# MohamedAbou-Taleb/Iterative-Linear-Quadratic-Regulator

Hardware: AMD Instinct MI355X
Metric: iLQR iterations/sec (batch=4096, T=200, n=4 m=1); backward-pass HBM GB/s (higher is better)
Workload: dtype f32; 1 GPU; c3: under-actuated double pendulum swing-up (run_iLQR_UA_MPC.py params), n=4 m=1 N=200 rk4, batch 4096 trajectories per GPU, 10 parallel line-search alphas per pass covering the 10 reference trials, fixed iterations; batch_per_gpu=4096, horizon=200, n_alpha=10, n_trials=10

## Files before the change

iterative-linear-quadratic-regulator_amd/csrc/backward_tile16.hpp:

```cpp
#pragma once
#include <type_traits>
#include <utility>

#include "dynamics.hpp"

namespace ilqr {

constexpr int dpp_quad(int a, int b, int c, int d) { return a | (b << 2) | (c << 4) | (d << 6); }
constexpr int kRowRor = 0x120;
constexpr int kDown1 = kRowRor + 12;
constexpr int kDown2 = kRowRor + 8;
constexpr int kDown3 = kRowRor + 4;
constexpr int kRight1 = dpp_quad(1, 2, 3, 0);
constexpr int kRight2 = dpp_quad(2, 3, 0, 1);
constexpr int kRight3 = dpp_quad(3, 0, 1, 2);
constexpr int kSwap1 = dpp_quad(1, 0, 3, 2);

template <int CTRL, int BANK = 0xf, bool BOUND = true> ILQR_DEV int dpp_bits(int old, int v) {
    return __builtin_amdgcn_update_dpp(old, v, CTRL, 0xf, BANK, BOUND);
}
template <int CTRL> ILQR_DEV float dpp(float v) {
    return __int_as_float(dpp_bits<CTRL>(0, __float_as_int(v)));
}
template <int CTRL> ILQR_DEV double dpp(double v) {
    const int lo = dpp_bits<CTRL>(0, __double2loint(v));
    const int hi = dpp_bits<CTRL>(0, __double2hiint(v));
    return __hiloint2double(hi, lo);
}
template <int CTRL, int BANK> ILQR_DEV float dpp_row(float old, float v) {
    return __int_as_float(dpp_bits<CTRL, BANK, false>(__float_as_int(old), __float_as_int(v)));
}
template <int CTRL, int BANK> ILQR_DEV double dpp_row(double old, double v) {
    const int lo = dpp_bits<CTRL, BANK, false>(__double2loint(old), __double2loint(v));
    const int hi = dpp_bits<CTRL, BANK, false>(__double2hiint(old), __double2hiint(v));
    return __hiloint2double(hi, lo);
}

template <typename T> struct Vec4;
template <> struct Vec4<float> { using type = float4; };
template <> struct Vec4<double> { using type = double4; };

constexpr int kTile16 = 48;

constexpr int kTileAux = ILQR_NT_TILE_LOAD ? 2 : 0;
typedef unsigned int u32x4 __attribute__((ext_vector_type(4)));
typedef unsigned int u32x2 __attribute__((ext_vector_type(2)));
ILQR_DEV int uniform(int v) { return __builtin_amdgcn_readfirstlane(v); }
ILQR_DEV __amdgpu_buffer_rsrc_t make_rsrc(const void* base, unsigned bytes) {
    const unsigned long long a = (unsigned long long)base;
    const unsigned lo = (unsigned)uniform((int)(unsigned)a), hi = (unsigned)uniform((int)(unsigned)(a >> 32));
    void* ub = (void*)(((unsigned long long)hi << 32) | lo);
    return __builtin_amdgcn_make_buffer_rsrc(ub, 0, (unsigned)uniform((int)bytes), 0x00020000);
}
template <int IMM, typename T> struct BufLoad;
template <int IMM> struct BufLoad<IMM, float> {
    static ILQR_DEV void v4(__amdgpu_buffer_rsrc_t r, int voff, int soff, float* o) {
        const u32x4 v = __builtin_amdgcn_raw_buffer_load_b128(r, voff + IMM * 4, soff, kTileAux);
        o[0] = __uint_as_float(v.x); o[1] = __uint_as_float(v.y); o[2] = __uint_as_float(v.z); o[3] = __uint_as_float(v.w);
    }
    static ILQR_DEV float v1(__amdgpu_buffer_rsrc_t r, int voff, int soff) {
        return __uint_as_float(__builtin_amdgcn_raw_buffer_load_b32(r, voff + IMM * 4, soff, kTileAux));
    }
};
template <int IMM> struct BufLoad<IMM, double> {
    static ILQR_DEV void v4(__amdgpu_buffer_rsrc_t r, int voff, int soff, double* o) {
        const u32x4 a = __builtin_amdgcn_raw_buffer_load_b128(r, voff + IMM * 8, soff, kTileAux);
        const u32x4 b = __builtin_amdgcn_raw_buffer_load_b128(r, voff + IMM * 8 + 16, soff, kTileAux);
        o[0] = __hiloint2double((int)a.y, (int)a.x); o[1] = __hiloint2double((int)a.w, (int)a.z);
        o[2] = __hiloint2double((int)b.y, (int)b.x); o[3] = __hiloint2double((int)b.w, (int)b.z);
    }
    static ILQR_DEV double v1(__amdgpu_buffer_rsrc_t r, int voff, int soff) {
        const u32x2 a = __builtin_amdgcn_raw_buffer_load_b64(r, voff + IMM * 8, soff, kTileAux);
        return __hiloint2double((int)a.y, (int)a.x);
    }
};
ILQR_DEV void buf_store1(__amdgpu_buffer_rsrc_t r, int voff, int soff, float v) {
    __builtin_amdgcn_raw_buffer_store_b32(__float_as_uint(v), r, voff, soff, 0);
}
ILQR_DEV void buf_store1(__amdgpu_buffer_rsrc_t r, int voff, int soff, double v) {
    u32x2 w = {(unsigned)__double2loint(v), (unsigned)__double2hiint(v)};
    __builtin_amdgcn_raw_buffer_store_b64(w, r, voff, soff, 0);
}

template <typename T, int C, bool NOP2 = false> ILQR_DEV void buf_store_vec(__amdgpu_buffer_rsrc_t r, int voff, int soff, const T* v) {
    constexpr int BYTES = C * (int)sizeof(T), PB = BYTES % 16 == 0 ? 16 : BYTES % 8 == 0 ? 8 : 4, NP = BYTES / PB;
    unsigned w[BYTES / 4];
    __builtin_memcpy(w, v, BYTES);
#pragma unroll
    for (int k = 0; k < NP; ++k) {
        if constexpr (PB == 16) {
            const u32x4 q = {w[4 * k], w[4 * k + 1], w[4 * k + 2], w[4 * k + 3]};
            __builtin_amdgcn_raw_buffer_store_b128(q, r, voff + 16 * k, soff, 0);
            if constexpr (NOP2) asm volatile("s_nop 1" : : "v"(q));
            else asm volatile("s_nop 0" : : "v"(q));
        } else if constexpr (PB == 8) {
            const u32x2 q = {w[2 * k], w[2 * k + 1]};
            __builtin_amdgcn_raw_buffer_store_b64(q, r, voff + 8 * k, soff, 0);
        } else {
            __builtin_amdgcn_raw_buffer_store_b32(w[k], r, voff + 4 * k, soff, 0);
        }
    }
}

struct TileOffsets { int vi, vj, vl; };

template <typename T> struct Tile16 {
    T ski[4];
    T skj[4];
    T vj[4];
    T lxx;
    T bi;
    T luxi;
};

template <typename T> ILQR_DEV void tile16_load(Tile16<T>& tl, const T* __restrict__ tp, int i, int j, int l16) {
    using V4 = typename Vec4<T>::type;
    const V4 a = *reinterpret_cast<const V4*>(tp + 4 * i);
    const V4 c = *reinterpret_cast<const V4*>(tp + 4 * j);
    const V4 v = *reinterpret_cast<const V4*>(tp + 32 + 4 * j);
    tl.ski[0] = a.x; tl.ski[1] = a.y; tl.ski[2] = a.z; tl.ski[3] = a.w;
    tl.skj[0] = c.x; tl.skj[1] = c.y; tl.skj[2] = c.z; tl.skj[3] = c.w;
    tl.vj[0] = v.x; tl.vj[1] = v.y; tl.vj[2] = v.z; tl.vj[3] = v.w;
    tl.lxx = tp[16 + l16];
    tl.bi = tp[32 + 4 * i];
    tl.luxi = tp[32 + 4 * i + 2];
}

template <typename T>
ILQR_DEV void tile16_load_buf(Tile16<T>& tl, __amdgpu_buffer_rsrc_t r, const TileOffsets& o, int soff) {
    BufLoad<0, T>::v4(r, o.vi, soff, tl.ski);
    BufLoad<0, T>::v4(r, o.vj, soff, tl.skj);
    BufLoad<32, T>::v4(r, o.vj, soff, tl.vj);
    tl.lxx = BufLoad<16, T>::v1(r, o.vl, soff);
    tl.bi = BufLoad<32, T>::v1(r, o.vi, soff);
    tl.luxi = BufLoad<34, T>::v1(r, o.vi, soff);
}

struct TileQ {
    float skj[4];
    float vj[4];
    float a;
    float lxx;
    float c;
};
ILQR_DEV void tileq_load_buf(TileQ& tl, __amdgpu_buffer_rsrc_t r, const TileOffsets& o, int soff) {
    BufLoad<0, float>::v4(r, o.vj, soff, tl.skj);
    BufLoad<32, float>::v4(r, o.vj, soff, tl.vj);
    tl.a = BufLoad<0, float>::v1(r, o.vl, soff);
    tl.lxx = BufLoad<16, float>::v1(r, o.vl, soff);
    tl.c = BufLoad<32, float>::v1(r, o.vl, soff);
}

#if ILQR_NT_TILE_LOAD
#define ILQR_TILE_NT " nt"
#else
#define ILQR_TILE_NT ""
#endif
typedef int i32x4 __attribute__((ext_vector_type(4)));
typedef float f32x4n __attribute__((ext_vector_type(4)));
typedef double f64x2n __attribute__((ext_vector_type(2)));

ILQR_DEV i32x4 make_srd(const void* base, unsigned bytes) {
    const unsigned long long a = (unsigned long long)base;
    i32x4 d;
    d.x = uniform((int)(unsigned)a);
    d.y = uniform((int)((unsigned)(a >> 32) & 0xffffu));
    d.z = uniform((int)bytes);
    d.w = 0x00020000;
    return d;
}

template <int... I, typename F> ILQR_DEV void static_for_impl(std::integer_sequence<int, I...>, F&& f) {
    (f(std::integral_constant<int, I>{}), ...);
}
template <int N, typename F> ILQR_DEV void static_for(F&& f) {
    static_for_impl(std::make_integer_sequence<int, N>{}, f);
}

template <typename T> struct RawTile;
#define ILQR_OUT_FIRST(x) "=&v"(x)
#define ILQR_OUT_REFILL(x) "+&v"(x)
template <> struct RawTile<float> {
    static constexpr int NLOAD = 5;
    f32x4n ski, skj, vj, vi;
    float lxx;
#define ILQR_RAWTILE_F32(OUT)                                                                \
    asm volatile(                                                                            \
        "s_nop 4\n\t"                                                                        \
        "buffer_load_dwordx4 %0, %5, %8, %9 offen" ILQR_TILE_NT "\n\t"                       \
        "buffer_load_dwordx4 %1, %6, %8, %9 offen" ILQR_TILE_NT "\n\t"                       \
        "buffer_load_dwordx4 %2, %6, %8, %9 offen offset:128" ILQR_TILE_NT "\n\t"            \
        "buffer_load_dword %3, %7, %8, %9 offen offset:64" ILQR_TILE_NT "\n\t"               \
        "buffer_load_dwordx4 %4, %5, %8, %9 offen offset:128" ILQR_TILE_NT                   \
        : OUT(ski), OUT(skj), OUT(vj), OUT(lxx), OUT(vi)                                     \
        : "v"(o.vi), "v"(o.vj), "v"(o.vl), "s"(srd), "s"(soff)                               \
        : "memory")
    template <bool FIRST> ILQR_DEV void issue(const i32x4& srd, const TileOffsets& o, int soff) {
        if constexpr (FIRST) ILQR_RAWTILE_F32(ILQR_OUT_FIRST);
        else ILQR_RAWTILE_F32(ILQR_OUT_REFILL);
    }
    template <int N> ILQR_DEV void wait() {
        asm volatile("s_waitcnt vmcnt(%5)" : "+v"(ski), "+v"(skj), "+v"(vj), "+v"(lxx), "+v"(vi) : "i"(N) : "memory");
    }
    ILQR_DEV void unpack(Tile16<float>& t) const {
        t.ski[0] = ski.x; t.ski[1] = ski.y; t.ski[2] = ski.z; t.ski[3] = ski.w;
// ... 599 lines not shown
```

iterative-linear-quadratic-regulator_amd/csrc/kernels.hpp:

```cpp
#pragma once
#include "dynamics.hpp"

namespace ilqr {

#ifndef ILQR_NT_TILE_STORE
#define ILQR_NT_TILE_STORE 0
#endif
#ifndef ILQR_NT_TILE_LOAD
#define ILQR_NT_TILE_LOAD 0
#endif
#ifndef ILQR_DROP_ALL
#define ILQR_DROP_ALL 0
#endif
constexpr int kMaxAlpha = 16;
constexpr int kCounterRing = 64;
constexpr int kBoxMaxU = 2;
constexpr int kALMaxX = 4;

template <typename T> struct Limits {
    T u_lo[kBoxMaxU], u_hi[kBoxMaxU];
    T x_lo[kALMaxX], x_hi[kALMaxX];
    int al_mask;
    const T* u_lo_rows;
    const T* u_hi_rows;
    const T* x_lo_rows;
    const T* x_hi_rows;
};

template <typename T> struct KArgs {
    int B, N, n_slots, integ, maxiter, flags;
    int n_pass;
    int last_pass;
    int init_mode;
    int counter_idx;
    T dt, tol, mu;
    T alphas[kMaxAlpha];
    T* X; T* U; int* cur_slot;
    T* gains; T* lin; T* term; T* x0;
    T* costs; T* cost; T* cost_prev; T* alpha_taken;
    int* status; int* iters; int* accepted; int* counters;
    int reset_slots;
    int const_lin;
    int fuse_select;
    int lin_sparse;
    int t_first;
    const T* params;
    long long* probe;
    alignas(sizeof(T)) int box;
    alignas(sizeof(T)) int het;
    const T* rows;
    const T* plant_rows;
    const T* lam;
    const T* rho;
    Limits<T> lim;
};

template <int NU, typename T> ILQR_DEV void box_bounds(const Limits<T>& a, size_t B, int b, T* lo, T* hi) {
    const T* __restrict__ rl = a.u_lo_rows;
    const T* __restrict__ rh = a.u_hi_rows;
#pragma unroll
    for (int j = 0; j < NU; ++j) {
        lo[j] = rl ? rl[(size_t)j * B + b] : a.u_lo[j];
        hi[j] = rl ? rh[(size_t)j * B + b] : a.u_hi[j];
    }
}

template <int NH, typename T> ILQR_DEV void load_row(T* p, const T* __restrict__ rows, size_t B, int b) {
#pragma unroll
    for (int q = 0; q < NH; ++q) p[q] = rows[(size_t)q * B + b];
}

constexpr int gain_record(int nx, int nu) { return ((nu * nx + nu) + 3) / 4 * 4; }

ILQR_DEV bool traj_active(int status) { return (status & 0xff) == ILQR_TRAJ_ACTIVE; }

template <typename T> ILQR_DEV T clamp_keep_nan(T v, T lo, T hi) { return v < lo ? lo : (v > hi ? hi : v); }

ILQR_DEV size_t vec_at(size_t B, int Tn, int C, int slot, int t, size_t b) {
    return ((((size_t)slot * Tn + t) * B) + b) * C;
}
typedef unsigned int vec_u4 __attribute__((ext_vector_type(4)));
typedef unsigned int vec_u2 __attribute__((ext_vector_type(2)));
constexpr int vec_piece(int bytes) { return bytes % 16 == 0 ? 16 : bytes % 8 == 0 ? 8 : 4; }
constexpr int vec_pieces(int bytes) { return bytes / vec_piece(bytes); }
template <typename T, int C> ILQR_DEV void vec_load(const T* __restrict__ p, T* o) {
    constexpr int BYTES = C * (int)sizeof(T), PB = vec_piece(BYTES), NP = BYTES / PB;
    if constexpr (PB == 16) {
        vec_u4 v[NP];
#pragma unroll
        for (int k = 0; k < NP; ++k) v[k] = reinterpret_cast<const vec_u4*>(p)[k];
        __builtin_memcpy(o, v, BYTES);
    } else if constexpr (PB == 8) {
        vec_u2 v[NP];
#pragma unroll
        for (int k = 0; k < NP; ++k) v[k] = reinterpret_cast<const vec_u2*>(p)[k];
        __builtin_memcpy(o, v, BYTES);
    } else {
#pragma unroll
        for (int i = 0; i < C; ++i) o[i] = p[i];
    }
}
template <typename T, int C> ILQR_DEV void vec_store(T* __restrict__ p, const T* v) {
    constexpr int BYTES = C * (int)sizeof(T), PB = vec_piece(BYTES), NP = BYTES / PB;
    if constexpr (PB == 16) {
        vec_u4 w[NP];
        __builtin_memcpy(w, v, BYTES);
#pragma unroll
        for (int k = 0; k < NP; ++k) reinterpret_cast<vec_u4*>(p)[k] = w[k];
    } else if constexpr (PB == 8) {
        vec_u2 w[NP];
        __builtin_memcpy(w, v, BYTES);
#pragma unroll
        for (int k = 0; k < NP; ++k) reinterpret_cast<vec_u2*>(p)[k] = w[k];
    } else {
#pragma unroll
        for (int i = 0; i < C; ++i) p[i] = v[i];
    }
}

struct ClockProbe {
    long long c0, r0;
    ILQR_DEV void start() { c0 = __builtin_readcyclecounter(); r0 = wall_clock64(); }
    ILQR_DEV void stop(long long* probe, int slot) const {
        if (probe && threadIdx.x == 0) {
            const long long c1 = __builtin_readcyclecounter(), r1 = wall_clock64();
            const size_t wg = (size_t)blockIdx.y * gridDim.x + blockIdx.x;
            if (wg == 0) { probe[2 * slot] = c1 - c0; probe[2 * slot + 1] = r1 - r0; }
            if (wg < 65536) {
                long long* q = probe + 8 + ((size_t)slot * 65536 + wg) * 4;
                q[0] = r0; q[1] = r1; q[2] = c1 - c0;
                q[3] = (long long)__builtin_amdgcn_s_getreg((4 ) | (0 << 6) | (31 << 11)) |
                       ((long long)__builtin_amdgcn_s_getreg((20 ) | (0 << 6) | (3 << 11)) << 32);
            }
        }
    }
};

}
#include "backward_tile16.hpp"
#include "backward_tile16m2.hpp"
namespace ilqr {

template <typename TS, int NX, int NU, typename T, typename Pick>
ILQR_DEV void tile16_fill(Pick pick, const T (*fx)[NX], const T (*fu)[NU], const T* gxn, const T* gu1, const T (*lxxn)[NX],
                          const T (*luxn)[NX], const T (*luu)[NU], typename Vec4<TS>::type* tile) {
    static_assert((NX >= 2 && NX <= 4 && NU == 1) || (NX == 4 && NU == 2), "tile packing: n_x <= 4 with n_u = 1, or (4, 2)");
    auto F = [&](int i, int j) -> TS { return (i < NX && j < NX) ? pick(fx[i < NX ? i : 0][j < NX ? j : 0]) : TS(0); };
    auto L = [&](int i, int j) -> TS { return (i < NX && j < NX) ? pick(lxxn[i < NX ? i : 0][j < NX ? j : 0]) : TS(0); };
#pragma unroll
    for (int c = 0; c < 4; ++c) {
        tile[c].x = F((c + 0) & 3, c); tile[c].y = F((c + 1) & 3, c);
        tile[c].z = F((c + 2) & 3, c); tile[c].w = F((c + 3) & 3, c);
    }
#pragma unroll
// ... 600 lines not shown
    if (a.reset_slots) a.cur_slot[b] = 0;
    const size_t B = a.B;
    T Vx[NX], Vxx[NX][NX];
    load_terminal<T, NX>(a.term, B, b, Vx, Vxx);
    bool all_pd = true;
    T blo[NU], bhi[NU];
    box_bounds<NU>(a.lim, a.B, b, blo, bhi);
    for (int t = a.N - 1; t >= 0; --t) {
        T tile[E], u[NU];
        load_expansion<E>(a.lin + ((size_t)t * E) * B + b, B, tile);
        vec_load<T, NU>(a.U + vec_at(B, a.N, NU, slot, t, b), u);
        T Qx[NX], Qu[NU], Qxx[NX][NX], Qux[NU][NX], Quu[NU][NU], Qr[NU][NU];
        riccati_q<T, NX, NU>(tile, Vx, Vxx, Qx, Qu, Qxx, Qux, Quu);
#pragma unroll
        for (int i = 0; i < NU; ++i)
#pragma unroll
            for (int j = 0; j < NU; ++j) Qr[i][j] = Quu[i][j] + ((i == j) ? a.mu : T(0));
        T K[NU][NX], k[NU], lo[NU], hi[NU];
        const bool pd = gain_solve<T, NX, NU>(Qr, Qux, Qu, K, k);
        all_pd = all_pd && pd;
#pragma unroll
        for (int i = 0; i < NU; ++i) {
            lo[i] = blo[i] - u[i];
            hi[i] = bhi[i] - u[i];
        }
        const bool moved = box_gains<T, NX, NU>(Qr, Qux, Qu, lo, hi, pd, K, k);
        riccati_value<T, NX, NU>(moved || a.mu != T(0), Qx, Qu, Qxx, Qux, Quu, K, k, Vx, Vxx);
        constexpr int R = gain_record(NX, NU);
        store_gains<T, NX, NU>(a.gains + ((size_t)t * B + b) * R, K, k);
    }
    if (!all_pd) a.status[b] = st | ILQR_TRAJ_FLAG_NON_PD;
}

template <typename T, typename Dyn, int INTEG, bool BOX, bool HET = false, bool AL = false>
ILQR_DEV void forward_body(const KArgs<T>& a) {
    constexpr int NX = Dyn::NX, NU = Dyn::NU;
    constexpr int R = gain_record(NX, NU);
    const int b = blockIdx.x * blockDim.x + threadIdx.x;
    const int ai = blockIdx.y;
    if (a.init_mode && blockIdx.x == 0 && ai == 0 && threadIdx.x == 0) a.counters[a.counter_idx] = 0;
    if (b >= a.B) return;
    if (!a.init_mode) {
        if (!traj_active(a.status[b])) return;
        if (a.accepted[b]) return;
    }
    const size_t B = a.B;
    const int N = a.N;
    const int slot = a.cur_slot[b];
    const int cslot = (slot + 1 + ai) % a.n_slots;
    const T alpha = a.alphas[ai];
    using PLf = ParamLayout<Dyn::NSYS, NX, NU>;
    T ph[HET ? PLf::QS : 1];
    if constexpr (HET) {
#pragma unroll
        for (int i = 0; i < PLf::QS; ++i) ph[i] = a.params[i];
        load_row<PLf::Q>(ph, a.rows, B, b);
    }
    const T* __restrict__ p = HET ? ph : a.params;
    T x[NX], u[NU];
#pragma unroll
    for (int i = 0; i < NX; ++i) x[i] = a.x0[(size_t)i * B + b];
    ClockProbe cp;
    cp.start();
    T cost = T(0);
    const T* Xo = a.X + vec_at(B, N + 1, NX, slot, 0, b);
    const T* Uo = a.U + vec_at(B, N, NU, slot, 0, b);
    const T* G = a.gains + (size_t)b * R;
    T* Xc = a.X + vec_at(B, N + 1, NX, cslot, 0, b);
    T* Uc = a.U + vec_at(B, N, NU, cslot, 0, b);
    const size_t sX = B * NX, sU = B * NU;
    constexpr bool PREFETCH = (R <= 32);
    constexpr int RN = PREFETCH ? R : 1, NXN = PREFETCH ? NX : 1, NUN = PREFETCH ? NU : 1;
    T xo[NX], uo[NU], g[R], xo_n[NXN], uo_n[NUN], g_n[RN];
    vec_load<T, NX>(Xo, xo);
    vec_load<T, NU>(Uo, uo);
#pragma unroll
    for (int r = 0; r < R; ++r) g[r] = G[r];
    constexpr int NL = AL ? 2 * NX : 1;
    T lam[NL], lam_n[NL];
    const T rho = AL ? a.rho[b] : T(0);
    T blo[BOX ? NU : 1], bhi[BOX ? NU : 1];
    if constexpr (BOX) box_bounds<NU>(a.lim, a.B, b, blo, bhi);
    struct NoBounds { ILQR_DEV NoBounds(const Limits<T>&, size_t, int) {} };
    const std::conditional_t<AL, ALBounds<T, NX>, NoBounds> xb(a.lim, a.B, b);
    for (int t = 0; t < N; ++t) {
        const int tn = (t + 1 < N) ? t + 1 : t;
        if constexpr (PREFETCH) {
            vec_load<T, NX>(Xo + tn * sX, xo_n);
            vec_load<T, NU>(Uo + tn * sU, uo_n);
#pragma unroll
            for (int r = 0; r < R; ++r) g_n[r] = G[(size_t)tn * B * R + r];
        }
        T dx[NX];
#pragma unroll
        for (int i = 0; i < NX; ++i) dx[i] = x[i] - xo[i];
#pragma unroll
        for (int j = 0; j < NU; ++j) {
            T fb = T(0);
#pragma unroll
            for (int i = 0; i < NX; ++i) fb += g[j * NX + i] * dx[i];
            u[j] = uo[j] + alpha * g[NU * NX + j] + fb;
            if constexpr (BOX) u[j] = clamp_keep_nan(u[j], blo[j], bhi[j]);
        }
        vec_store<T, NX>(Xc + t * sX, x);
        vec_store<T, NU>(Uc + t * sU, u);
        cost += Cost<T, Dyn>::stage(p, a.dt, x, u);
        if constexpr (AL) {
            if (t > 0) cost += al_phi<T, NX>(xb, x, lam, rho);
            al_load_lam<T, NX>(a, B, b, t + 1, lam_n);
        }
        T xn[NX];
        Stepper<T, Dyn>::step(INTEG, p, a.dt, x, u, xn);
#pragma unroll
        for (int i = 0; i < NX; ++i) x[i] = xn[i];
        if constexpr (AL) {
#pragma unroll
            for (int q = 0; q < NL; ++q) lam[q] = lam_n[q];
        }
        if constexpr (PREFETCH) {
#pragma unroll
            for (int i = 0; i < NX; ++i) xo[i] = xo_n[i];
#pragma unroll
            for (int j = 0; j < NU; ++j) uo[j] = uo_n[j];
#pragma unroll
            for (int r = 0; r < R; ++r) g[r] = g_n[r];
        } else {
            vec_load<T, NX>(Xo + tn * sX, xo);
            vec_load<T, NU>(Uo + tn * sU, uo);
#pragma unroll
            for (int r = 0; r < R; ++r) g[r] = G[(size_t)tn * B * R + r];
        }
    }
    vec_store<T, NX>(Xc + N * sX, x);
    cost += Cost<T, Dyn>::terminal(p, x);
    if constexpr (AL) cost += al_phi<T, NX>(xb, x, lam, rho);
    a.costs[(size_t)ai * B + b] = cost;
    cp.stop(a.probe, 1);
}
template <typename T, typename Dyn, int INTEG>
__global__ void __launch_bounds__(64) forward_kernel(KArgs<T> a) { forward_body<T, Dyn, INTEG, false>(a); }
template <typename T, typename Dyn, int INTEG>
__global__ void __launch_bounds__(64) forward_kernel_box(KArgs<T> a) { forward_body<T, Dyn, INTEG, true>(a); }
template <typename T, typename Dyn, int INTEG>
__global__ void __launch_bounds__(64) forward_kernel_het(KArgs<T> a) { forward_body<T, Dyn, INTEG, false, true>(a); }
template <typename T, typename Dyn, int INTEG>
__global__ void __launch_bounds__(64) forward_kernel_box_het(KArgs<T> a) { forward_body<T, Dyn, INTEG, true, true>(a); }
template <typename T, typename Dyn, int INTEG>
__global__ void __launch_bounds__(64) forward_kernel_al(KArgs<T> a) { forward_body<T, Dyn, INTEG, true, false, true>(a); }
template <typename T, typename Dyn, int INTEG>
__global__ void __launch_bounds__(64) forward_kernel_al_het(KArgs<T> a) { forward_body<T, Dyn, INTEG, true, true, true>(a); }

#include "fwd_in_gen.inc"

template <typename T, typename Dyn, int INTEG, bool BOX = false, bool HET = false>
ILQR_DEV void rollout_ring(const KArgs<T>& a, int b, int ai, bool in_range, bool force_init = false) {
    constexpr int NX = Dyn::NX, NU = Dyn::NU;
    using In = FwdIn<T, NX, NU>;
    constexpr int R = In::R, NLD = In::NLD, NST = vec_pieces(NX * (int)sizeof(T)) + vec_pieces(NU * (int)sizeof(T));
#ifndef ILQR_RING_PF_MAX
#define ILQR_RING_PF_MAX 6
#endif
    constexpr int SLOT_REGS = (NX + NU + R) * (int)sizeof(T) / 4;
    constexpr int PF_CNT = (63 / (NLD + NST)) + 1 > ILQR_RING_PF_MAX ? ILQR_RING_PF_MAX : (63 / (NLD + NST)) + 1;
    constexpr int RING_CAP = ((sizeof(T) == 8 && INTEG == ILQR_INT_BACKWARD_EULER) ? 104 : 130) -
                             (HET ? (Dyn::NSYS + NX) * (int)sizeof(T) / 4 : 0) -
                             ((BOX && HET && sizeof(T) == 8 && INTEG == ILQR_INT_EULER) ? SLOT_REGS : 0);
    constexpr int PF = PF_CNT * SLOT_REGS > RING_CAP ? RING_CAP / SLOT_REGS : PF_CNT;
    static_assert(PF >= 2, "ring too shallow to be worth it");
    const int bc = in_range ? b : 0;
    ai = in_range ? ai : 0;
    const int st_raw = a.status[bc], acc_raw = a.accepted[bc], slot_raw = a.cur_slot[bc];
    const bool live = in_range & ((a.init_mode != 0) | force_init | (traj_active(st_raw) & (acc_raw == 0)));
    if (__ballot(live) == 0ull) return;
    const int bb = live ? b : 0;
    const size_t B = a.B;
    const int N = a.N;
    const int slot = slot_raw;
    const int cslot = (slot + 1 + ai) % a.n_slots;
    const T alpha = force_init ? T(0) : a.alphas[ai];
    const T dt = a.dt;
    T lo[NU], hi[NU];
    if constexpr (BOX) {
        box_bounds<NU>(a.lim, a.B, bb, lo, hi);
    } else {
#pragma unroll
        for (int j = 0; j < NU; ++j) lo[j] = hi[j] = T(0);
    }
    using PLp = ParamLayout<Dyn::NSYS, NX, NU>;
    T p[PLp::QS];
#pragma unroll
    for (int i = 0; i < PLp::QS; ++i) p[i] = a.params[i];
    if constexpr (HET) load_row<PLp::Q>(p, a.rows, B, bb);
    T x[NX], u[NU];
#pragma unroll
    for (int i = 0; i < NX; ++i) x[i] = a.x0[(size_t)i * B + bb];
    ClockProbe cp;
    cp.start();
    T cost = T(0);
    const int stepX = (int)(B * NX * sizeof(T)), stepU = (int)(B * NU * sizeof(T)), stepG = (int)(B * R * sizeof(T));
    const unsigned bytesX = (unsigned)((size_t)a.n_slots * (N + 1) * NX * B * sizeof(T));
    const unsigned bytesU = (unsigned)((size_t)a.n_slots * N * NU * B * sizeof(T));
    const __amdgpu_buffer_rsrc_t rXc = make_rsrc(a.X, bytesX), rUc = make_rsrc(a.U, bytesU);
    constexpr bool DROP = sizeof(T) == 4 || ILQR_DROP_ALL;
    const int kDropped = 0x7ffffff0;
    const int vXc = (live || !DROP) ? (int)(vec_at(B, N + 1, NX, cslot, 0, bb) * sizeof(T)) : kDropped;
    const int vUc = (live || !DROP) ? (int)(vec_at(B, N, NU, cslot, 0, bb) * sizeof(T)) : kDropped;
    const __amdgpu_buffer_rsrc_t srdG = make_rsrc(a.gains, (unsigned)((size_t)N * B * R * sizeof(T)));
    const int vx = (int)(vec_at(B, N + 1, NX, slot, 0, bb) * sizeof(T));
    const int vu = (int)(vec_at(B, N, NU, slot, 0, bb) * sizeof(T));
    const int vg = (int)((size_t)bb * R * sizeof(T));
    auto issue = [&](In& in, int t, auto first) {
        in.template issue<decltype(first)::value>(rXc, rUc, srdG, vx, vu, vg, t * stepX, t * stepU, t * stepG);
    };
    constexpr std::true_type kFirst{};
    constexpr std::false_type kRefill{};
    auto do_step = [&](const In& in, int t) {
        T xo[NX], uo[NU], dx[NX];
        in.unpack(xo, uo);
#ifndef ILQR_NO_CTRL_PK
        if constexpr (sizeof(T) == 4 && NX == 4) {
            typedef float f2 __attribute__((ext_vector_type(2)));
            auto pair = [](float a, float b) { f2 r; r.x = a; r.y = b; return r; };
            const f2 d01 = pair(x[0], x[1]) - pair(xo[0], xo[1]), d23 = pair(x[2], x[3]) - pair(xo[2], xo[3]);
#pragma unroll
            for (int j = 0; j < NU; ++j) {
                const f2 f = __builtin_elementwise_fma(pair(in.gain(j * NX + 2), in.gain(j * NX + 3)), d23,
                                                       pair(in.gain(j * NX + 0), in.gain(j * NX + 1)) * d01);
                u[j] = uo[j] + alpha * in.gain(NU * NX + j) + (f.x + f.y);
            }
        } else
#endif
        {
#pragma unroll
        for (int i = 0; i < NX; ++i) dx[i] = x[i] - xo[i];
#pragma unroll
        for (int j = 0; j < NU; ++j) {
            T fb = T(0);
#pragma unroll
            for (int i = 0; i < NX; ++i) fb += in.gain(j * NX + i) * dx[i];
            u[j] = uo[j] + alpha * in.gain(NU * NX + j) + fb;
        }
        }
        if constexpr (BOX) {
#pragma unroll
            for (int j = 0; j < NU; ++j) u[j] = clamp_keep_nan(u[j], lo[j], hi[j]);
        }
        if (DROP || live) {
            buf_store_vec<T, NX, HET>(rXc, vXc, uniform(t * stepX), x);
            buf_store_vec<T, NU, HET>(rUc, vUc, uniform(t * stepU), u);
        }
        cost += Cost<T, Dyn>::stage(p, dt, x, u);
        T xn[NX];
        Stepper<T, Dyn>::step(INTEG, p, dt, x, u, xn);
#pragma unroll
        for (int i = 0; i < NX; ++i) x[i] = xn[i];
    };
    int t = 0;
    for (int r = N % PF; r > 0; --r, ++t) {
        In in;
        issue(in, t, kFirst);
        in.template wait<0>();
        do_step(in, t);
    }
    if (t < N) {
        In ring[PF];
#pragma unroll
        for (int q = 0; q < PF; ++q) issue(ring[q], t + q, kFirst);
#pragma unroll
        for (int q = 0; q < PF; ++q) {
            ring[q].template wait<(PF - 1) * NLD>();
            do_step(ring[q], t + q);
            issue(ring[q], (t + q + PF < N) ? t + q + PF : N - 1, kRefill);
        }
        for (t += PF; t < N; t += PF) {
#pragma unroll
            for (int q = 0; q < PF; ++q) {
                ring[q].template wait<(PF - 1) * (NLD + NST)>();
                do_step(ring[q], t + q);
                issue(ring[q], (t + q + PF < N) ? t + q + PF : N - 1, kRefill);
            }
        }
        asm volatile("s_waitcnt vmcnt(0)" ::: "memory");
    }
    if (live) {
        vec_store<T, NX>(a.X + vec_at(B, N + 1, NX, cslot, N, bb), x);
        cost += Cost<T, Dyn>::terminal(p, x);
        a.costs[(size_t)ai * B + b] = cost;
    }
    cp.stop(a.probe, 1);
}

template <typename T, typename Dyn, int INTEG>
__global__ void __launch_bounds__(64) forward_ring_kernel(KArgs<T> a) {
    const int b = blockIdx.x * blockDim.x + threadIdx.x;
    const int ai = blockIdx.y;
    if (a.init_mode && blockIdx.x == 0 && ai == 0 && threadIdx.x == 0) a.counters[a.counter_idx] = 0;
    rollout_ring<T, Dyn, INTEG>(a, b, ai, b < a.B);
}
template <typename T, typename Dyn, int INTEG>
__global__ void __launch_bounds__(64) forward_ring_kernel_box(KArgs<T> a) {
    const int b = blockIdx.x * blockDim.x + threadIdx.x;
    const int ai = blockIdx.y;
    if (a.init_mode && blockIdx.x == 0 && ai == 0 && threadIdx.x == 0) a.counters[a.counter_idx] = 0;
    rollout_ring<T, Dyn, INTEG, true>(a, b, ai, b < a.B);
}
template <typename T, typename Dyn, int INTEG>
__global__ void __launch_bounds__(64) forward_ring_kernel_het(KArgs<T> a) {
    const int b = blockIdx.x * blockDim.x + threadIdx.x;
    const int ai = blockIdx.y;
    if (a.init_mode && blockIdx.x == 0 && ai == 0 && threadIdx.x == 0) a.counters[a.counter_idx] = 0;
    rollout_ring<T, Dyn, INTEG, false, true>(a, b, ai, b < a.B);
}
template <typename T, typename Dyn, int INTEG>
__global__ void __launch_bounds__(64) forward_ring_kernel_box_het(KArgs<T> a) {
    const int b = blockIdx.x * blockDim.x + threadIdx.x;
    const int ai = blockIdx.y;
    if (a.init_mode && blockIdx.x == 0 && ai == 0 && threadIdx.x == 0) a.counters[a.counter_idx] = 0;
    rollout_ring<T, Dyn, INTEG, true, true>(a, b, ai, b < a.B);
}

template <typename T>
ILQR_DEV bool select_candidates(const KArgs<T>& a, int b, bool last_pass, int& slot_out, int& status_out) {
    const size_t B = a.B;
    int st = a.status[b];
    int slot = a.cur_slot[b];
    const int acc_in = a.accepted[b];
    const T c0 = a.cost[b];
    T cs[kMaxAlpha];
#pragma unroll
    for (int ai = 0; ai < kMaxAlpha; ++ai) cs[ai] = ai < a.n_pass ? a.costs[(size_t)ai * B + b] : T(0);
    const int it_in = a.iters[b];
    const T cp_in = a.cost_prev[b];
    T cost_now = c0, cost_before = cp_in;
    bool still_active = false;
    if (traj_active(st)) {
        int acc = acc_in;
        if (!acc) {
            int first = -1;
#pragma unroll
            for (int ai = kMaxAlpha - 1; ai >= 0; --ai)
                if (ai < a.n_pass && cs[ai] <= c0) first = ai;
            if (first >= 0) {
                T c = cs[0], al = a.alphas[0];
#pragma unroll
                for (int ai = 1; ai < kMaxAlpha; ++ai)
                    if (ai == first) { c = cs[ai]; al = a.alphas[ai]; }
                slot = (slot + 1 + first) % a.n_slots;
                a.cost_prev[b] = c0;
                a.cost[b] = c;
                a.alpha_taken[b] = al;
                cost_now = c;
                cost_before = c0;
                acc = 1;
            }
        }
        if (last_pass) {
            const int it = it_in + 1;
            a.iters[b] = it;
            a.accepted[b] = 0;
            if (!(a.flags & ILQR_FLAG_KEEP_ITERATING)) {
                if (!acc) {
                    st = (st & ~0xff) | ILQR_TRAJ_LINESEARCH_FAILED;
                } else if (it >= a.maxiter) {
                    st = (st & ~0xff) | ILQR_TRAJ_MAXITER;
                } else {
                    const T d = M<T>::abs(cost_now - cost_before);
                    if (d <= a.tol) st = (st & ~0xff) | ILQR_TRAJ_CONVERGED;
                }
                a.status[b] = st;
            }
            if (!acc) a.alpha_taken[b] = T(0);
        } else {
            a.accepted[b] = acc;
        }
        still_active = traj_active(st);
    }
    slot_out = slot;
    status_out = st;
    return still_active;
}

template <typename T>
__global__ void __launch_bounds__(256) select_kernel(KArgs<T> a) {
    const int b = blockIdx.x * blockDim.x + threadIdx.x;
    bool still_active = false;
    if (b < a.B) {
        if (a.init_mode) {
            const T c = a.costs[b];
            a.cur_slot[b] = (a.cur_slot[b] + 1) % a.n_slots;
            a.cost[b] = c;
            a.cost_prev[b] = c;
            a.alpha_taken[b] = T(0);
            a.status[b] = ILQR_TRAJ_ACTIVE;
            a.iters[b] = 0;
            a.accepted[b] = 0;
            still_active = true;
        } else {
            int slot, st;
            const int slot_before = a.cur_slot[b];
            still_active = select_candidates(a, b, a.last_pass != 0, slot, st);
            if (slot != slot_before) a.cur_slot[b] = slot;
        }
    }
    if (a.last_pass || a.init_mode) {
        const unsigned long long m = __ballot(still_active);
        if ((threadIdx.x & 63) == 0 && m) atomicAdd(&a.counters[a.counter_idx], (int)__popcll(m));
        if (blockIdx.x == 0 && threadIdx.x == 0) a.counters[(a.counter_idx + 1) % kCounterRing] = 0;
    }
}

template <typename T> struct ALArgs {
    T* lam;
    T* rho;
    T* viol;
    T* cost_plain;
    int* outer;
    int* live;
    int* base;
    int* count;
    T ctol, rho0, rho_factor, rho_max;
    int max_outer;
};

template <typename T>
__global__ void __launch_bounds__(256) al_reset_kernel(ALArgs<T> s, int B) {
    const int b = blockIdx.x * blockDim.x + threadIdx.x;
    if (b >= B) return;
    s.rho[b] = s.rho0;
    s.viol[b] = T(0);
    s.outer[b] = 0;
    s.live[b] = 1;
    s.base[b] = 0;
}

template <typename T, typename Dyn, bool HET> struct CostParams {
    using PL = ParamLayout<Dyn::NSYS, Dyn::NX, Dyn::NU>;
    T ph[HET ? PL::QS : 1];
    const T* p;
    ILQR_DEV CostParams(const KArgs<T>& a, int b) {
        if constexpr (HET) {
#pragma unroll
            for (int i = 0; i < PL::QS; ++i) ph[i] = a.params[i];
            load_row<PL::Q>(ph, a.rows, (size_t)a.B, b);
        }
        p = HET ? ph : a.params;
    }
};

template <typename T, typename Dyn> ILQR_DEV T plain_cost(const T* p, T dt, const T* Xb, const T* Ub, size_t B, int N) {
    constexpr int NX = Dyn::NX, NU = Dyn::NU;
    T cost = T(0);
    for (int t = 0; t < N; ++t) {
        T x[NX], u[NU];
        vec_load<T, NX>(Xb + t * (B * NX), x);
        vec_load<T, NU>(Ub + t * (B * NU), u);
        cost += Cost<T, Dyn>::stage(p, dt, x, u);
    }
    T x[NX];
    vec_load<T, NX>(Xb + N * (B * NX), x);
    return cost + Cost<T, Dyn>::terminal(p, x);
}

template <typename T, typename Dyn, bool HET = false>
__global__ void __launch_bounds__(64) al_update_kernel(KArgs<T> a, ALArgs<T> s) {
    constexpr int NX = Dyn::NX, NU = Dyn::NU;
    const int b = blockIdx.x * blockDim.x + threadIdx.x;
    bool rearm = false;
    if (b < a.B && s.live[b]) {
        const size_t B = a.B;
        const int N = a.N;
        const int slot = a.cur_slot[b];
// ... 352 lines not shown
```

iterative-linear-quadratic-regulator_amd/systems/custom_sys.py:

```python
from __future__ import annotations

import hashlib
import os
import shutil
import subprocess

import numpy as np

from .. import _lib
from .system_base import System

PLUGIN_ROOT = os.path.join(_lib.HERE, "_plugins")
TEMPLATE = os.path.join(_lib.CSRC, "plugin_template.hip.in")
_KERNEL_HEADERS = ("dynamics.hpp", "kernels.hpp", "backward_tile16.hpp", "backward_tile16m2.hpp", "tile16m2_step_gen.inc", "backward_fused16.hpp",
                   "persistent.hpp", "forward_mfma16.hpp", "kernels_wave.hpp", "backward_mfma16.hpp", "fwd_in_gen.inc", "policy_rollout.hpp", "sample_controls.hpp", "sampled_mpc.hpp",
                   "ops.hpp", "solver.hpp", "plugin_template.hip.in", "check_ring_kernels.py", "verify_ring_isa.py")


def _ring_check():
    import importlib.util
    spec = importlib.util.spec_from_file_location("ilqr_check_ring_kernels", os.path.join(_lib.CSRC, "check_ring_kernels.py"))
    mod = importlib.util.module_from_spec(spec)
    spec.loader.exec_module(mod)
    return mod


def _printer(n_x, n_u):
    from sympy.printing.c import C99CodePrinter

    class DevicePrinter(C99CodePrinter):
        _ns = "um::"

        def _print_Float(self, e):
            return f"T({float(e)!r})"

        def _print_Rational(self, e):
            return f"T({int(e.p)}.0 / {int(e.q)}.0)"

        def _print_Integer(self, e):
            return f"T({int(e)})"

        def _print_NumberSymbol(self, e):
            return f"T({float(e.evalf(17))!r})"

        _print_Pi = _print_Exp1 = _print_NumberSymbol

        def _print_Pow(self, e):
            base, ex = e.base, e.exp
            b = self.parenthesize(base, 1000)
            if ex.is_Integer and 1 <= abs(int(ex)) <= 4:
                prod = " * ".join([b] * abs(int(ex)))
                return f"({prod})" if int(ex) > 0 else f"um::rcp({prod})"
            if ex == sp_half():
                return f"um::sqrt({self._print(base)})"
            if ex == -sp_half():
                return f"(T(1) / um::sqrt({self._print(base)}))"
            return f"um::pow({self._print(base)}, {self._print(ex)})"

    return DevicePrinter()


def sp_half():
    import sympy as sp
    return sp.Rational(1, 2)


def _trace_symbols(n_x, n_u):
    import sympy as sp
    xs = sp.symbols(f"x_0:{n_x}", real=True)
    us = sp.symbols(f"u_0:{n_u}", real=True)
    names = {**{s: f"x[{i}]" for i, s in enumerate(xs)}, **{s: f"u[{i}]" for i, s in enumerate(us)}}
    pr = _printer(n_x, n_u)
    pr._print_Symbol = lambda s: names.get(s, s.name)

    def block(targets):
        exprs = [e for _, e in targets]
        sums = {f: sp.expand_trig(f) for e in exprs for f in e.atoms(sp.sin, sp.cos) if f.args[0].is_Add}
        if sums:
            exprs = [e.xreplace(sums) for e in exprs]
        args = []
        for e in exprs:
            for f in e.atoms(sp.sin, sp.cos):
                a = f.args[0]
                if a.free_symbols <= set(xs) | set(us) and not a.atoms(sp.sin, sp.cos) and a not in args:
                    args.append(a)
        args.sort(key=sp.default_sort_key)
        trig = {}
        for k, a in enumerate(args):
            trig[sp.sin(a)] = sp.Symbol(f"sn_{k}", real=True)
            trig[sp.cos(a)] = sp.Symbol(f"cs_{k}", real=True)
        exprs = [e.xreplace(trig) for e in exprs]
        lines = []
        if args:
            lines.append("        T " + ", ".join(f"sn_{k}, cs_{k}" for k in range(len(args))) + ";")
            for k in range(0, len(args) - 1, 2):
                lines.append(f"        um::sincos2({pr.doprint(args[k])}, {pr.doprint(args[k + 1])}, &sn_{k}, &cs_{k}, "
                             f"&sn_{k + 1}, &cs_{k + 1});")
            if len(args) % 2:
                k = len(args) - 1
                lines.append(f"        um::sincos({pr.doprint(args[k])}, &sn_{k}, &cs_{k});")
        repl, red = sp.cse(exprs, symbols=sp.numbered_symbols("w_"), optimizations="basic")
        lines += [f"        const T {pr.doprint(s)} = {pr.doprint(e)};" for s, e in repl]
        lines += [f"        {name} = {pr.doprint(e)};" for (name, _), e in zip(targets, red)]
        return "\n".join(lines)

    def check_free(exprs, what):
        free = set().union(*[e.free_symbols for e in exprs]) - set(xs) - set(us)
        if free:
            raise ValueError(f"{what} has free symbols other than x, u: {sorted(map(str, free))}")

    return xs, us, block, check_free


def generate_dyn_bodies(f_cont, n_x, n_u):
    import sympy as sp
    xs, us, block, check_free = _trace_symbols(n_x, n_u)
    out = f_cont(list(xs), list(us))
    out = [sp.sympify(e) for e in (out.tolist() if hasattr(out, "tolist") else list(out))]
    out = [e[0] if isinstance(e, (list, tuple)) else e for e in out]
    if len(out) != n_x:
        raise ValueError(f"_f_cont_fcn returned {len(out)} components, expected n_x = {n_x}")
    check_free(out, "_f_cont_fcn")
    nq = n_x // 2
    generate_dyn_bodies.second_order = n_x % 2 == 0 and all(sp.simplify(out[i] - xs[nq + i]) == 0 for i in range(nq))
    f_targets = [(f"xd[{i}]", e) for i, e in enumerate(out)]
    jac = list(f_targets)
    jac += [(f"Jx[{i}][{j}]", sp.diff(out[i], xs[j])) for i in range(n_x) for j in range(n_x)]
    jac += [(f"Ju[{i}][{j}]", sp.diff(out[i], us[j])) for i in range(n_x) for j in range(n_u)]
    return block(f_targets), block(jac)


def generate_cost_bodies(l_fcn, l_f_fcn, n_x, n_u):
    import sympy as sp
    xs, us, block, check_free = _trace_symbols(n_x, n_u)
    l = sp.sympify(l_fcn(list(xs), list(us)))
    lf = sp.sympify(l_f_fcn(list(xs)))
    check_free([l], "_l_fcn")
    check_free([lf], "_l_f_fcn")
    if lf.free_symbols & set(us):
        raise ValueError("_l_f_fcn must depend on x only")
    d = [(f"lx[{i}]", sp.diff(l, xs[i])) for i in range(n_x)] + [(f"lu[{j}]", sp.diff(l, us[j])) for j in range(n_u)]
    d += [(f"lxx[{i}][{j}]", sp.diff(l, xs[i], xs[j])) for i in range(n_x) for j in range(n_x)]
    d += [(f"lux[{j}][{i}]", sp.diff(l, us[j], xs[i])) for j in range(n_u) for i in range(n_x)]
    d += [(f"luu[{i}][{j}]", sp.diff(l, us[i], us[j])) for i in range(n_u) for j in range(n_u)]
    df = [(f"g[{i}]", sp.diff(lf, xs[i])) for i in range(n_x)]
    df += [(f"H[{i}][{j}]", sp.diff(lf, xs[i], xs[j])) for i in range(n_x) for j in range(n_x)]
    return block([("out", l)]), block(d), block([("out", lf)]), block(df)


def render_plugin_source(f_cont, n_x, n_u, dtype, l_fcn=None, l_f_fcn=None, policy_kernels=False):
    f_body, fjac_body = generate_dyn_bodies(f_cont, n_x, n_u)
    if l_fcn is not None:
        cost = generate_cost_bodies(l_fcn, l_f_fcn, n_x, n_u)
    else:
        cost = ("        out = T(0);", "", "        out = T(0);", "")
    src = open(TEMPLATE).read()
    for key, val in (("@NX@", str(n_x)), ("@NU@", str(n_u)), ("@F_BODY@", f_body), ("@FJAC_BODY@", fjac_body),
                     ("@SECOND_ORDER@", "true" if generate_dyn_bodies.second_order else "false"),
                     ("@CUSTOM_COST@", "true" if l_fcn is not None else "false"),
                     ("@L_BODY@", cost[0]), ("@L_DERIVS_BODY@", cost[1]), ("@LF_BODY@", cost[2]),
                     ("@LF_DERIVS_BODY@", cost[3]),
                     ("@DTYPE@", "float" if np.dtype(dtype) == np.float32 else "double")):
        src = src.replace(key, val)
    if policy_kernels:
        src = "#define ILQR_PLUGIN_POLICY 1\n" + src
    return src

# ... 122 lines not shown
```

Before: 29.74 million iLQR iterations/sec.

## Rebase buffer descriptors per ring pass and pin params and offsets in SGPRs

Restructures the f32 forward ring rollout so each pass advances the buffer resource base addresses instead of computing per-step scalar offsets, using fixed per-slot offsets kept in SGPRs. Uniform cost parameters are pinned into scalar registers, and the last ring pass gets its own exact waitcnt values. The goal is to cut scalar and vector address arithmetic and register pressure in the rollout's inner loop. It adds descriptor rebuilding every pass and more complex schedule code, with a risk of SGPR pressure.

```diff
diff --git a/iterative-linear-quadratic-regulator_amd/csrc/backward_tile16.hpp b/iterative-linear-quadratic-regulator_amd/csrc/backward_tile16.hpp
--- a/iterative-linear-quadratic-regulator_amd/csrc/backward_tile16.hpp
+++ b/iterative-linear-quadratic-regulator_amd/csrc/backward_tile16.hpp
@@ -51,6 +51,14 @@
     const unsigned lo = (unsigned)uniform((int)(unsigned)a), hi = (unsigned)uniform((int)(unsigned)(a >> 32));
     void* ub = (void*)(((unsigned long long)hi << 32) | lo);
     return __builtin_amdgcn_make_buffer_rsrc(ub, 0, (unsigned)uniform((int)bytes), 0x00020000);
+}
+ILQR_DEV unsigned long long uniform_addr(const void* base) {
+    const unsigned long long a = (unsigned long long)base;
+    const unsigned lo = (unsigned)uniform((int)(unsigned)a), hi = (unsigned)uniform((int)(unsigned)(a >> 32));
+    return ((unsigned long long)hi << 32) | lo;
+}
+ILQR_DEV __amdgpu_buffer_rsrc_t make_rsrc_at(unsigned long long uniform_address, unsigned uniform_bytes) {
+    return __builtin_amdgcn_make_buffer_rsrc((void*)uniform_address, 0, uniform_bytes, 0x00020000);
 }
 template <int IMM, typename T> struct BufLoad;
 template <int IMM> struct BufLoad<IMM, float> {
diff --git a/iterative-linear-quadratic-regulator_amd/csrc/kernels.hpp b/iterative-linear-quadratic-regulator_amd/csrc/kernels.hpp
--- a/iterative-linear-quadratic-regulator_amd/csrc/kernels.hpp
+++ b/iterative-linear-quadratic-regulator_amd/csrc/kernels.hpp
@@ -1,5 +1,6 @@
 #pragma once
 #include "dynamics.hpp"
+#include "ring_plan.hpp"
 
 namespace ilqr {
 
@@ -906,7 +907,7 @@
 
 #include "fwd_in_gen.inc"
 
-template <typename T, typename Dyn, int INTEG, bool BOX = false, bool HET = false>
+template <typename T, typename Dyn, int INTEG, bool BOX = false, bool HET = false, bool SCALAR_ARGS = false>
 ILQR_DEV void rollout_ring(const KArgs<T>& a, int b, int ai, bool in_range, bool force_init = false) {
     constexpr int NX = Dyn::NX, NU = Dyn::NU;
     using In = FwdIn<T, NX, NU>;
@@ -921,6 +922,7 @@
                              ((BOX && HET && sizeof(T) == 8 && INTEG == ILQR_INT_EULER) ? SLOT_REGS : 0);
     constexpr int PF = PF_CNT * SLOT_REGS > RING_CAP ? RING_CAP / SLOT_REGS : PF_CNT;
     static_assert(PF >= 2, "ring too shallow to be worth it");
+    constexpr bool PLAN = SCALAR_ARGS && sizeof(T) == 4;
     const int bc = in_range ? b : 0;
     ai = in_range ? ai : 0;
     const int st_raw = a.status[bc], acc_raw = a.accepted[bc], slot_raw = a.cur_slot[bc];
@@ -945,6 +947,10 @@
 #pragma unroll
     for (int i = 0; i < PLp::QS; ++i) p[i] = a.params[i];
     if constexpr (HET) load_row<PLp::Q>(p, a.rows, B, bb);
+    if constexpr (PLAN) {
+#pragma unroll
+        for (int i = (HET ? PLp::Q : 0); i < PLp::QS; ++i) asm("" : "+s"(p[i]));
+    }
     T x[NX], u[NU];
 #pragma unroll
     for (int i = 0; i < NX; ++i) x[i] = a.x0[(size_t)i * B + bb];
@@ -954,21 +960,21 @@
     const int stepX = (int)(B * NX * sizeof(T)), stepU = (int)(B * NU * sizeof(T)), stepG = (int)(B * R * sizeof(T));
     const unsigned bytesX = (unsigned)((size_t)a.n_slots * (N + 1) * NX * B * sizeof(T));
     const unsigned bytesU = (unsigned)((size_t)a.n_slots * N * NU * B * sizeof(T));
-    const __amdgpu_buffer_rsrc_t rXc = make_rsrc(a.X, bytesX), rUc = make_rsrc(a.U, bytesU);
+    __amdgpu_buffer_rsrc_t rXc = make_rsrc(a.X, bytesX), rUc = make_rsrc(a.U, bytesU);
+    __amdgpu_buffer_rsrc_t srdG = make_rsrc(a.gains, (unsigned)((size_t)N * B * R * sizeof(T)));
     constexpr bool DROP = sizeof(T) == 4 || ILQR_DROP_ALL;
     const int kDropped = 0x7ffffff0;
     const int vXc = (live || !DROP) ? (int)(vec_at(B, N + 1, NX, cslot, 0, bb) * sizeof(T)) : kDropped;
     const int vUc = (live || !DROP) ? (int)(vec_at(B, N, NU, cslot, 0, bb) * sizeof(T)) : kDropped;
-    const __amdgpu_buffer_rsrc_t srdG = make_rsrc(a.gains, (unsigned)((size_t)N * B * R * sizeof(T)));
     const int vx = (int)(vec_at(B, N + 1, NX, slot, 0, bb) * sizeof(T));
     const int vu = (int)(vec_at(B, N, NU, slot, 0, bb) * sizeof(T));
     const int vg = (int)((size_t)bb * R * sizeof(T));
-    auto issue = [&](In& in, int t, auto first) {
-        in.template issue<decltype(first)::value>(rXc, rUc, srdG, vx, vu, vg, t * stepX, t * stepU, t * stepG);
+    auto issue = [&](In& in, int vx_, int vu_, int vg_, int sx, int su, int sg, auto first) {
+        in.template issue<decltype(first)::value>(rXc, rUc, srdG, vx_, vu_, vg_, sx, su, sg);
     };
     constexpr std::true_type kFirst{};
     constexpr std::false_type kRefill{};
-    auto do_step = [&](const In& in, int t) {
+    auto do_step = [&](const In& in, int sx, int su) {
         T xo[NX], uo[NU], dx[NX];
         in.unpack(xo, uo);
 #ifndef ILQR_NO_CTRL_PK
@@ -1000,8 +1006,8 @@
             for (int j = 0; j < NU; ++j) u[j] = clamp_keep_nan(u[j], lo[j], hi[j]);
         }
         if (DROP || live) {
-            buf_store_vec<T, NX, HET>(rXc, vXc, uniform(t * stepX), x);
-            buf_store_vec<T, NU, HET>(rUc, vUc, uniform(t * stepU), u);
+            buf_store_vec<T, NX, HET || PLAN>(rXc, vXc, uniform(sx), x);
+            buf_store_vec<T, NU, HET || PLAN>(rUc, vUc, uniform(su), u);
         }
         cost += Cost<T, Dyn>::stage(p, dt, x, u);
         T xn[NX];
@@ -1009,32 +1015,87 @@
 #pragma unroll
         for (int i = 0; i < NX; ++i) x[i] = xn[i];
     };
-    int t = 0;
-    for (int r = N % PF; r > 0; --r, ++t) {
-        In in;
-        issue(in, t, kFirst);
-        in.template wait<0>();
-        do_step(in, t);
-    }
-    if (t < N) {
+    if constexpr (PLAN) {
+        RingOffsets<PF> oX(uniform_addr(a.X), uniform(stepX)), oU(uniform_addr(a.U), uniform(stepU)),
+            oG(uniform_addr(a.gains), uniform(stepG));
+        auto pin = [&] {
+#pragma unroll
+            for (int q = 1; q < PF; ++q) {
+                asm("" : "+s"(oX.slot[q]));
+                asm("" : "+s"(oU.slot[q]));
+                asm("" : "+s"(oG.slot[q]));
+            }
+        };
+        const unsigned recX = (unsigned)uniform((int)bytesX), recU = (unsigned)uniform((int)bytesU),
+                       recG = (unsigned)uniform((int)(unsigned)((size_t)N * B * R * sizeof(T)));
+        auto rebase = [&] {
+            rXc = make_rsrc_at(oX.base, recX);
+            rUc = make_rsrc_at(oU.base, recU);
+            srdG = make_rsrc_at(oG.base, recG);
+        };
+        const int vx_ahead = vx + oX.pass(), vu_ahead = vu + oU.pass(), vg_ahead = vg + oG.pass();
+        using Waits = RingWaits<PF, NLD, NST>;
         In ring[PF];
-#pragma unroll
-        for (int q = 0; q < PF; ++q) issue(ring[q], t + q, kFirst);
-#pragma unroll
-        for (int q = 0; q < PF; ++q) {
-            ring[q].template wait<(PF - 1) * NLD>();
-            do_step(ring[q], t + q);
-            issue(ring[q], (t + q + PF < N) ? t + q + PF : N - 1, kRefill);
-        }
-        for (t += PF; t < N; t += PF) {
+        ring_walk<PF>(
+            N,
+            [&] {
+                In in;
+                issue(in, vx, vu, vg, oX.at(0), oU.at(0), oG.at(0), kFirst);
+                in.template wait<0>();
+                do_step(in, oX.at(0), oU.at(0));
+            },
+            [&](int steps) {
+                oX.advance(steps);
+                oU.advance(steps);
+                oG.advance(steps);
+                rebase();
+            },
+            [&](auto q) { issue(ring[q], vx, vu, vg, oX.at(q), oU.at(q), oG.at(q), kFirst); },
+            [&](auto q, int r) {
+                ring[q].template wait<Waits::first>();
+                do_step(ring[q], oX.at(q), oU.at(q));
+                issue(ring[q], vx, vu, vg, oX.behind(r), oU.behind(r), oG.behind(r), kRefill);
+            },
+            pin,
+            [&](auto q) {
+                ring[q].template wait<Waits::steady>();
+                do_step(ring[q], oX.at(q), oU.at(q));
+                issue(ring[q], vx_ahead, vu_ahead, vg_ahead, oX.at(q), oU.at(q), oG.at(q), kRefill);
+            },
+            [&](auto q) {
+                ring[q].template wait<Waits::last(q)>();
+                do_step(ring[q], oX.at(q), oU.at(q));
+            },
+            [] { asm volatile("s_waitcnt vmcnt(0)" ::: "memory"); });
+    } else {
+        int t = 0;
+        auto at = [&](In& in, int step, auto first) { issue(in, vx, vu, vg, step * stepX, step * stepU, step * stepG, first); };
+        for (int r = N % PF; r > 0; --r, ++t) {
+            In in;
+            at(in, t, kFirst);
+            in.template wait<0>();
+            do_step(in, t * stepX, t * stepU);
+        }
+        if (t < N) {
+            In ring[PF];
+#pragma unroll
+            for (int q = 0; q < PF; ++q) at(ring[q], t + q, kFirst);
 #pragma unroll
             for (int q = 0; q < PF; ++q) {
-                ring[q].template wait<(PF - 1) * (NLD + NST)>();
-                do_step(ring[q], t + q);
-                issue(ring[q], (t + q + PF < N) ? t + q + PF : N - 1, kRefill);
-            }
-        }
-        asm volatile("s_waitcnt vmcnt(0)" ::: "memory");
+                ring[q].template wait<(PF - 1) * NLD>();
+                do_step(ring[q], (t + q) * stepX, (t + q) * stepU);
+                at(ring[q], (t + q + PF < N) ? t + q + PF : N - 1, kRefill);
+            }
+            for (t += PF; t < N; t += PF) {
+#pragma unroll
+                for (int q = 0; q < PF; ++q) {
+                    ring[q].template wait<(PF - 1) * (NLD + NST)>();
+                    do_step(ring[q], (t + q) * stepX, (t + q) * stepU);
+                    at(ring[q], (t + q + PF < N) ? t + q + PF : N - 1, kRefill);
+                }
+            }
+            asm volatile("s_waitcnt vmcnt(0)" ::: "memory");
+        }
     }
     if (live) {
         vec_store<T, NX>(a.X + vec_at(B, N + 1, NX, cslot, N, bb), x);
@@ -1049,28 +1110,28 @@
     const int b = blockIdx.x * blockDim.x + threadIdx.x;
     const int ai = blockIdx.y;
     if (a.init_mode && blockIdx.x == 0 && ai == 0 && threadIdx.x == 0) a.counters[a.counter_idx] = 0;
-    rollout_ring<T, Dyn, INTEG>(a, b, ai, b < a.B);
+    rollout_ring<T, Dyn, INTEG, false, false, true>(a, b, ai, b < a.B);
 }
 template <typename T, typename Dyn, int INTEG>
 __global__ void __launch_bounds__(64) forward_ring_kernel_box(KArgs<T> a) {
     const int b = blockIdx.x * blockDim.x + threadIdx.x;
     const int ai = blockIdx.y;
     if (a.init_mode && blockIdx.x == 0 && ai == 0 && threadIdx.x == 0) a.counters[a.counter_idx] = 0;
-    rollout_ring<T, Dyn, INTEG, true>(a, b, ai, b < a.B);
+    rollout_ring<T, Dyn, INTEG, true, false, true>(a, b, ai, b < a.B);
 }
 template <typename T, typename Dyn, int INTEG>
 __global__ void __launch_bounds__(64) forward_ring_kernel_het(KArgs<T> a) {
     const int b = blockIdx.x * blockDim.x + threadIdx.x;
     const int ai = blockIdx.y;
     if (a.init_mode && blockIdx.x == 0 && ai == 0 && threadIdx.x == 0) a.counters[a.counter_idx] = 0;
-    rollout_ring<T, Dyn, INTEG, false, true>(a, b, ai, b < a.B);
+    rollout_ring<T, Dyn, INTEG, false, true, true>(a, b, ai, b < a.B);
 }
 template <typename T, typename Dyn, int INTEG>
 __global__ void __launch_bounds__(64) forward_ring_kernel_box_het(KArgs<T> a) {
     const int b = blockIdx.x * blockDim.x + threadIdx.x;
     const int ai = blockIdx.y;
     if (a.init_mode && blockIdx.x == 0 && ai == 0 && threadIdx.x == 0) a.counters[a.counter_idx] = 0;
-    rollout_ring<T, Dyn, INTEG, true, true>(a, b, ai, b < a.B);
+    rollout_ring<T, Dyn, INTEG, true, true, true>(a, b, ai, b < a.B);
 }
 
 template <typename T>
diff --git a/iterative-linear-quadratic-regulator_amd/csrc/ring_plan.hpp b/iterative-linear-quadratic-regulator_amd/csrc/ring_plan.hpp
--- /dev/null
+++ b/iterative-linear-quadratic-regulator_amd/csrc/ring_plan.hpp
@@ -0,0 +1,73 @@
+#pragma once
+#include <type_traits>
+#include <utility>
+
+#if defined(__HIPCC__)
+#define ILQR_HD __host__ __device__ __forceinline__
+#else
+#define ILQR_HD inline
+#endif
+
+namespace ilqr {
+
+template <int PF> struct RingOffsets {
+    unsigned long long base;
+    int stride;
+    int slot[PF];
+    ILQR_HD constexpr RingOffsets(unsigned long long origin, int stride_) : base(origin), stride(stride_), slot{} {
+        for (int q = 0; q < PF; ++q) slot[q] = q * stride_;
+    }
+    ILQR_HD constexpr void advance(int steps) {
+        base = (base + (unsigned long long)((long long)steps * stride)) & 0xffffffffffffull;
+    }
+    ILQR_HD constexpr int at(int q) const { return slot[q]; }
+    ILQR_HD constexpr int pass() const { return PF * stride; }
+    ILQR_HD constexpr int behind(int r) const { return r * stride; }
+};
+
+struct RingSchedule {
+    int lead, steady;
+    bool ring, last;
+};
+ILQR_HD constexpr RingSchedule ring_schedule(int N, int PF) {
+    const int passes = N / PF;
+    return RingSchedule{N % PF, passes > 2 ? passes - 2 : 0, passes >= 1, passes >= 2};
+}
+ILQR_HD constexpr int ring_first_refill(int t0, int q, int N, int PF) { return t0 + q + PF < N ? t0 + q + PF : N - 1; }
+
+template <int PF, int NLD, int NST> struct RingWaits {
+    static constexpr int first = (PF - 1) * NLD;
+    static constexpr int steady = (PF - 1) * (NLD + NST);
+    static constexpr int last(int q) { return (PF - 1 - q) * (NLD + NST) + q * NST; }
+};
+
+template <class F, int... Q> ILQR_HD constexpr void ring_slots_seq(F&& f, std::integer_sequence<int, Q...>) {
+    (f(std::integral_constant<int, Q>{}), ...);
+}
+template <int PF, class F> ILQR_HD constexpr void ring_slots(F&& f) { ring_slots_seq(f, std::make_integer_sequence<int, PF>{}); }
+
+template <int PF, class Single, class Advance, class Prologue, class First, class Settle, class Steady, class Last, class Drain>
+ILQR_HD constexpr void ring_walk(int N, Single&& single, Advance&& advance, Prologue&& prologue, First&& first, Settle&& settle,
+                                 Steady&& steady, Last&& last, Drain&& drain) {
+    const RingSchedule s = ring_schedule(N, PF);
+    for (int r = s.lead; r > 0; --r) {
+        single();
+        advance(1);
+    }
+    if (!s.ring) return;
+    ring_slots<PF>(prologue);
+    const int t0 = s.lead;
+    ring_slots<PF>([&](auto q) { first(q, ring_first_refill(t0, q, N, PF) - t0); });
+    settle();
+    for (int m = s.steady; m > 0; --m) {
+        advance(PF);
+        ring_slots<PF>(steady);
+    }
+    if (s.last) {
+        advance(PF);
+        ring_slots<PF>(last);
+    }
+    drain();
+}
+
+}
diff --git a/iterative-linear-quadratic-regulator_amd/systems/custom_sys.py b/iterative-linear-quadratic-regulator_amd/systems/custom_sys.py
--- a/iterative-linear-quadratic-regulator_amd/systems/custom_sys.py
+++ b/iterative-linear-quadratic-regulator_amd/systems/custom_sys.py
@@ -12,7 +12,7 @@
 
 PLUGIN_ROOT = os.path.join(_lib.HERE, "_plugins")
 TEMPLATE = os.path.join(_lib.CSRC, "plugin_template.hip.in")
-_KERNEL_HEADERS = ("dynamics.hpp", "kernels.hpp", "backward_tile16.hpp", "backward_tile16m2.hpp", "tile16m2_step_gen.inc", "backward_fused16.hpp",
+_KERNEL_HEADERS = ("dynamics.hpp", "ring_plan.hpp", "kernels.hpp", "backward_tile16.hpp", "backward_tile16m2.hpp", "tile16m2_step_gen.inc", "backward_fused16.hpp",
                    "persistent.hpp", "forward_mfma16.hpp", "kernels_wave.hpp", "backward_mfma16.hpp", "fwd_in_gen.inc", "policy_rollout.hpp", "sample_controls.hpp", "sampled_mpc.hpp",
                    "ops.hpp", "solver.hpp", "plugin_template.hip.in", "check_ring_kernels.py", "verify_ring_isa.py")
 
```

After: 29.57 million iLQR iterations/sec. Within noise of the previous version (-0.6%).
